# delldu/VSTNet

Hardware: AMD Instinct MI355X
Metric: stylized frames/sec at 1024x1024 (1/2/4/8 GPU) + % HBM roofline (higher is better)
Workload: dtype bf16x3

## Files before the change

include/vstnet.h:

```cpp
#ifndef VSTNET_H
#define VSTNET_H

#include <stddef.h>
#include <stdint.h>

#ifdef __cplusplus
extern "C" {
#endif
#pragma GCC visibility push(default)

#define VST_OK 0
#define VST_E_ARG (-1)
#define VST_E_SHAPE (-2)
#define VST_E_MODE (-3)
#define VST_E_WORKSPACE (-4)

#define VST_PREC_BF16X3 0
#define VST_PREC_FP32 1
#define VST_PREC_F16X2 2

#define VST_PREC_F16X2H 3

#define VST_NUM_BLOCKS 32

// ... 100 lines not shown
                     int Cin, int Cout, int H, int W, int K, int stride, void* stream);
int vst_generic_squeeze(const float* x, float* y, int B, int D, int H, int W, void* stream);
int vst_generic_unsqueeze(const float* y, float* x, int B, int D, int H, int W, void* stream);
int vst_generic_copy_channels(const float* src, float* dst, int B, int C_src, int c0, int n, long HW, int C_dst, int d0,
                              void* stream);
int vst_generic_zero(float* dst, size_t n_floats, void* stream);

size_t vst_cwct_stats_f64_workspace_bytes(int N, long L);
int vst_cwct_stats_f64(const float* x, int N, long L, const uint8_t* mask, int label, double* stats, void* workspace,
                       void* stream);
size_t vst_cwct_factor_f64_workspace_bytes(int N);
int vst_cwct_factor_f64(const double* content_stats, const double* const* style_stats_host_array, const float* alphas_host,
                        int n_styles, float alpha_c, float eps, int N, double* affine, int* info, void* workspace,
                        void* stream);
int vst_cwct_apply_f64(const float* x, float* y, int N, long L, const double* affine, const uint8_t* mask, int label,
                       void* stream);

size_t vst_cwct_stats_n_workspace_bytes(int N, long L);
int vst_cwct_stats_n(const float* x, int N, long L, const uint8_t* mask, int label, double* stats, void* workspace,
                     size_t workspace_bytes, void* stream);
size_t vst_cwct_factor_n_workspace_bytes(int N);
int vst_cwct_factor_n(const double* content_stats, const double* const* style_stats_host_array, const float* alphas_host,
                      int n_styles, float alpha_c, float eps, int N, float* affine, int* info, void* workspace,
                      size_t workspace_bytes, void* stream);
int vst_cwct_prefactor_n(const double* stats, int N, float eps, double* out, int* info, void* workspace, size_t workspace_bytes,
                         void* stream);
int vst_cwct_apply_n(const float* x, float* y, int N, long L, const float* affine, const uint8_t* mask, int label, void* stream);
size_t vst_cwct_stats_n_f64_workspace_bytes(int N, long L);
int vst_cwct_stats_n_f64(const float* x, int N, long L, const uint8_t* mask, int label, double* stats, void* workspace,
                         size_t workspace_bytes, void* stream);
size_t vst_cwct_factor_n_f64_workspace_bytes(int N);
int vst_cwct_factor_n_f64(const double* content_stats, const double* const* style_stats_host_array, const float* alphas_host,
                          int n_styles, float alpha_c, float eps, int N, double* affine, int* info, void* workspace,
                          size_t workspace_bytes, void* stream);
int vst_cwct_apply_n_f64(const float* x, float* y, int N, long L, const double* affine, const uint8_t* mask, int label,
                         void* stream);

#define VST_KERNEL_ID(cin, cout, stride) (((cin) << 16) | ((cout) << 4) | (stride))
#define VST_KERNEL_ALL (-1)
#define VST_KERNEL_PACK 1
#define VST_KERNEL_UNPACK 2
#define VST_KERNEL_SPREAD 3
#define VST_KERNEL_GATHER 4
#define VST_KERNEL_CWCT_STATS 5
#define VST_KERNEL_CWCT_FACTOR 6
#define VST_KERNEL_CWCT_APPLY 7
#define VST_KERNEL_PRESPLIT 8
int vst_profile_begin(int kernel_id, int max_records);
int vst_profile_end(double* total_ms, int* launches);
int vst_profile_end_table(int* ids, double* ms, int* launches, int cap, int* n_ids);

#define VST_OPT_STAGE3_LEAN 1
#define VST_OPT_STAGE3_PINGPONG 2
int vst_set_option(int option, int value);
int vst_get_option(int option);

#pragma GCC visibility pop
#ifdef __cplusplus
}
#endif
#endif
```

vstnet_amd/_lib.py:

```python
from __future__ import annotations

import ctypes as C
import glob
import os
import subprocess

PKG_DIR = os.path.dirname(os.path.abspath(__file__))
REPO_DIR = os.path.dirname(PKG_DIR)
LIB_PATH = os.environ.get("VSTNET_HIP_LIB") or os.path.join(PKG_DIR, "libvstnet_hip.so")
RESOURCES_PATH = os.path.join(PKG_DIR, "libvstnet_hip.resources.txt")
SOURCES = sorted(glob.glob(os.path.join(PKG_DIR, "csrc", "*.hip")))
HEADERS = sorted(glob.glob(os.path.join(PKG_DIR, "csrc", "*.h"))) + [os.path.join(REPO_DIR, "include", "vstnet.h")]

NUM_BLOCKS = 32
PREC_BF16X3 = 0
PREC_FP32 = 1
PREC_F16X2 = 2
PREC_F16X2H = 3

EXPORTS = [
    "vst_version", "vst_error_string", "vst_conv_packed_bytes", "vst_pack_conv", "vst_pack_input",
    "vst_unpack_output", "vst_pack_input_u8", "vst_unpack_output_u8", "vst_revnet_forward_u8", "vst_revnet_inverse_u8",
    "vst_spread", "vst_gather", "vst_block_tmp_bytes", "vst_block_apply",
    "vst_pass_workspace_bytes", "vst_revnet_forward", "vst_revnet_inverse",
    "vst_cwct_stats_workspace_bytes", "vst_cwct_stats", "vst_cwct_factor", "vst_cwct_apply", "vst_cwct_apply_prec",
    "vst_cwct_prefactor", "vst_label_plan", "vst_cwct_labels_workspace_bytes", "vst_cwct_stats_labels",
    "vst_cwct_factor_labels", "vst_cwct_apply_labels", "vst_profile_begin", "vst_profile_end", "vst_profile_end_table", "vst_lab_luminance",
    "vst_revnet_encode", "vst_revnet_encode_u8", "vst_revnet_decode", "vst_revnet_decode_u8", "vst_code_to_z", "vst_z_to_code",
    "vst_cwct_stats_code_workspace_bytes", "vst_cwct_stats_code", "vst_cwct_apply_code",
    "vst_mask_to_code", "vst_cwct_stats_labels_code_workspace_bytes", "vst_cwct_stats_labels_code", "vst_cwct_apply_labels_code",
    "vst_revnet_decode_labels", "vst_revnet_decode_labels_u8", "vst_pass_sub_batch",
    "vst_normalize_block", "vst_range_flags", "vst_range_flags_async",
    "vst_cwct_stats_f64_workspace_bytes", "vst_cwct_stats_f64", "vst_cwct_factor_f64_workspace_bytes", "vst_cwct_factor_f64",
    "vst_cwct_apply_f64",
    "vst_generic_conv", "vst_generic_squeeze", "vst_generic_unsqueeze", "vst_generic_copy_channels", "vst_generic_zero",
    "vst_set_option", "vst_get_option",
    "vst_cwct_stats_n_workspace_bytes", "vst_cwct_stats_n", "vst_cwct_factor_n_workspace_bytes", "vst_cwct_factor_n",
    "vst_cwct_prefactor_n", "vst_cwct_apply_n", "vst_cwct_stats_n_f64_workspace_bytes", "vst_cwct_stats_n_f64",
    "vst_cwct_factor_n_f64_workspace_bytes", "vst_cwct_factor_n_f64", "vst_cwct_apply_n_f64",
]
OPT_STAGE3_LEAN = 1
OPT_STAGE3_PINGPONG = 2
RANGE_SATURATED = 1
RANGE_WEIGHT = 2


PRECISIONS = {"bf16x3": PREC_BF16X3, "fp32": PREC_FP32, "f16x2": PREC_F16X2, "f16x2h": PREC_F16X2H}


def default_precision() -> str:
    p = os.environ.get("VST_PRECISION", "bf16x3")
    if p not in PRECISIONS:
        raise ValueError(f"VST_PRECISION must be one of {sorted(PRECISIONS)}")
    return p


class VstError(RuntimeError):
    pass


class ConvWeights(C.Structure):
    _fields_ = [("packed", C.c_void_p), ("bias", C.c_void_p)]


class BlockWeights(C.Structure):
    _fields_ = [("conv", ConvWeights * 3)]


class NetWeights(C.Structure):
    _fields_ = [("blocks", BlockWeights * NUM_BLOCKS)]


def build(force: bool = False, verbose: bool = False) -> str:
    newest_src = max(os.path.getmtime(p) for p in SOURCES + HEADERS)
    if not force and os.path.exists(LIB_PATH) and os.path.getmtime(LIB_PATH) >= newest_src:
        return LIB_PATH
    hipcc = os.environ.get("HIPCC", "/opt/rocm/bin/hipcc")
    cmd = [hipcc, "-O3", "--offload-arch=gfx950", "-fPIC", "-shared", "-std=c++17", "-Xarch_host", "-fvisibility=hidden",
           "-I", os.path.join(REPO_DIR, "include"), "-o", LIB_PATH] + SOURCES
    cmd[1:1] = ["-Rpass-analysis=kernel-resource-usage", "-fno-caret-diagnostics"]
    if verbose:
        print(" ".join(cmd))
    p = subprocess.run(cmd, stderr=subprocess.PIPE, text=True)
    remarks = [ln.split("remark:", 1)[1].split("[-Rpass")[0].strip() for ln in p.stderr.splitlines() if "remark:" in ln]
    other = "\n".join(ln for ln in p.stderr.splitlines() if "remark:" not in ln and "kernel-resource-usage" not in ln)
    if p.returncode != 0:
        raise subprocess.CalledProcessError(p.returncode, cmd, stderr=other)
    if other.strip():
        print(other)
    table, name = [], None
    for r in remarks:
        if r.startswith("Function Name:"):
            name = r.split(":", 1)[1].strip()
        elif name and (r.startswith("VGPRs:") or r.startswith("ScratchSize") or r.startswith("LDS Size") or r.startswith("Occupancy")):
            table.append(f"{name}\t{r}")
# ... 162 lines not shown
```

vstnet_amd/csrc/conv.hip:

```cpp
#include <mutex>
#include <stdlib.h>
#include "common.h"

#ifndef VST_ABLATE
#define VST_ABLATE 0
#endif

struct ConvArgs {
    const float* in;
    float* out;
    const unsigned char* packed;
    const float* bias;
    int Hin, Win, Hout, Wout;
    int Wq;
    size_t in_img_stride;
    size_t out_img_stride;
    float sign;
    int tiles_x, tiles_y, tiles_total;
    const unsigned char* packed1;
    const float* bias1;
    unsigned char* out_sp;
    size_t out_sp_img_bytes;
    unsigned trace_base;
};
// ... 675 lines not shown
    for (int m = 0; m < C::MR; ++m)
#pragma unroll
        for (int n = 0; n < C::NB; ++n) acc[m][n] = f32x4{0.f, 0.f, 0.f, 0.f};
    const int slot_base = (wave * C::MR) * C::IW + lrow;
#pragma unroll
    for (int ks = 0; ks < C::KS; ++ks) {
        bf16x8 wh[C::NB], wl[C::NB];
#pragma unroll
        for (int n = 0; n < C::NB; ++n) {
            const int boff = ((ks * 4 + kg) * C::NT + n * 16 + lrow) * 16;
            wh[n] = __builtin_bit_cast(bf16x8, *(const uint4*)(b_hi + boff));
            wl[n] = __builtin_bit_cast(bf16x8, *(const uint4*)(b_lo + boff));
        }
#pragma unroll
        for (int m = 0; m < C::MR; ++m) {
            bf16x8 xh, xl;
            read_x_small<MID>(a_hi, a_lo, C::NSLOT, slot_base + m * C::IW, C::IW, ks, kg, xh, xl);
#pragma unroll
            for (int n = 0; n < C::NB; ++n) { MFMA_T(acc[m][n], wh[n], wl[n], xh, xl); }
        }
    }
    load_bias<CH, C::NB>(a, 4 * kg, bias);
    if constexpr (TERMS == 2) vst_note_range(range_amax);
    if (!EARLY_OLD) { PAIR_FETCH_OLD(); }
#undef PAIR_FETCH_OLD
    if (interior) store_tile<CH, true, C::MR, C::NB, true>(a, out_img, ty0 + wave * C::MR, tx0 + lrow, 4 * kg, acc, bias, old);
    else store_tile<CH, true, C::MR, C::NB>(a, out_img, ty0 + wave * C::MR, tx0 + lrow, 4 * kg, acc, bias, old);
    VST_TRACE_END_(1, MID, CH)
}

#ifdef VST_PP_STAMP
__device__ unsigned long long vst_pp_stamps[2 * 32 * 8];
extern "C" __attribute__((visibility("default"))) int vst_pp_stamps_dump(unsigned long long* host) {
    return (int)hipMemcpyFromSymbol(host, HIP_SYMBOL(vst_pp_stamps), sizeof(vst_pp_stamps));
}
#define PP_STAMP(grp_, st_, k_)                                                                                  \
    if (blockIdx.x == 128 && lane == 0 && (wave & 3) == 0 && (st_) < 32) {                                       \
        asm volatile("s_waitcnt lgkmcnt(0)" ::: "memory");                                                      \
        vst_pp_stamps[((grp_) * 32 + (st_)) * 8 + (k_)] = __builtin_amdgcn_s_memtime();                          \
    }
__device__ unsigned long long vst_pp_clk[4];
extern "C" __attribute__((visibility("default"))) int vst_pp_clk_dump(unsigned long long* host) {
    return (int)hipMemcpyFromSymbol(host, HIP_SYMBOL(vst_pp_clk), sizeof(vst_pp_clk));
}
#define PP_CLK(i_)                                                                                               \
    if (blockIdx.x == 128 && threadIdx.x == 0) {                                                                 \
        vst_pp_clk[2 * (i_)] = __builtin_amdgcn_s_memtime();                                                     \
        vst_pp_clk[2 * (i_) + 1] = __builtin_amdgcn_s_memrealtime();                                             \
    }
#else
#define PP_STAMP(grp_, st_, k_)
#define PP_CLK(i_)
#endif
template <int CIN, int COUT, int NW_ = 8>
struct PipeCfg {
    static constexpr int NW = NW_, NTHR = 64 * NW;
    static constexpr int NT = 64, NB = 4, MR = 2, TH = MR * NW, IW = 18, NPIX = (TH + 2) * IW, NSLOT = (NPIX + 15) / 16 * 16;
    static constexpr int NCHUNK = CIN / 32, NCOT = COUT / 64;
    static constexpr int A_PLANE = 4 * NSLOT * 16, A_BUF = 2 * A_PLANE;
    static constexpr int B_PLANE = 3 * 4 * 64 * 16, B_BUF = 2 * B_PLANE;
    static constexpr int LDS_BYTES = 2 * A_BUF + 2 * B_BUF;
    static constexpr int A_PART = NPIX * 4 / 3;
    static constexpr int A_ITEMS = ((A_PART / 4 + 15) / 16 * 64 + NTHR - 1) / NTHR;
    static constexpr int B_ITEMS = 2 * 768 / NTHR;
    static_assert(NPIX % 3 == 0, "three equal parts");
};

template <int CIN, int COUT, bool IN_STATE, bool OUT_STATE, int NW = 8>
__global__ __launch_bounds__(64 * NW, NW == 4 ? 2 : 1) void conv_pipe_kernel(const ConvArgs a) {
    using C = PipeCfg<CIN, COUT, NW>;
    extern __shared__ __attribute__((aligned(16))) unsigned char smem[];
    unsigned char* const Abuf = smem;
    unsigned char* const Bbuf = smem + 2 * C::A_BUF;

    const int tid = threadIdx.x, lane = tid & 63, wave = tid >> 6;
    const int lrow = lane & 15, kg = lane >> 4;
    int bx, by, b;
    if (!xcd_tile(a, bx, by, b)) return;
    VST_TRACE_BEGIN(4)
    PP_CLK(0)
    const int tx0 = bx * 16, ty0 = by * C::TH;
    const float* const in_img = a.in + (size_t)b * a.in_img_stride;
    float* const out_img = a.out + (size_t)b * a.out_img_stride;
    const PackedConvLayout PL = packed_conv_layout(COUT, CIN);
    const unsigned char* const w_plane0 = a.packed + PL.f32_bytes;

    unsigned a_src[3][C::A_ITEMS], a_dst[3][C::A_ITEMS];
#pragma unroll
    for (int part = 0; part < 3; ++part)
#pragma unroll
        for (int it = 0; it < C::A_ITEMS; ++it) {
            const int j = it * C::NTHR + tid;
            int sl = (j >> 6) * 16 + (j & 15);
            sl = sl < C::A_PART / 4 ? sl : C::A_PART / 4 - 1;
            const int cig = (j >> 4) & 3, slot = part * (C::A_PART / 4) + sl;
            const int iy = slot / C::IW, ix = slot - iy * C::IW;
            const int gy = reflect_clamp(ty0 - 1 + iy, a.Hin), gx = reflect_clamp(tx0 - 1 + ix, a.Win);
            const size_t off = IN_STATE ? zc_offset(vst_level_of_channels(CIN), gy, gx, a.Wq)
                                        : ((size_t)gy * a.Win + gx) * CIN;
            a_src[part][it] = (unsigned)(off + cig * 8);
            a_dst[part][it] = (cig * C::NSLOT + slot) * 16;
        }
    typedef f32x4 APart[C::A_ITEMS][2];
    typedef u32x4 BStage[C::B_ITEMS];
#define LOAD_A(r, chunk, part)                                                          \
    _Pragma("unroll") for (int it_ = 0; it_ < C::A_ITEMS; ++it_) {                      \
        const float* p_ = in_img + a_src[part][it_] + (chunk) * 32;                     \
        r[it_][0] = *(const f32x4*)p_; r[it_][1] = *(const f32x4*)(p_ + 4);             \
    }
#define F4_(v_) make_float4((v_)[0], (v_)[1], (v_)[2], (v_)[3])
#define STORE_A(buf, part, r)                                                           \
    _Pragma("unroll") for (int it_ = 0; it_ < C::A_ITEMS; ++it_) {                      \
        unsigned char* base_ = Abuf + (buf) * C::A_BUF;                                 \
        uint4 h_, l_;                                                                   \
        split8(F4_(r[it_][0]), F4_(r[it_][1]), h_, l_);                                 \
        *(uint4*)(base_ + a_dst[part][it_]) = h_;                                       \
        *(uint4*)(base_ + C::A_PLANE + a_dst[part][it_]) = l_;                          \
    }
    int b_off[C::B_ITEMS], b_dst[C::B_ITEMS];
#pragma unroll
    for (int it = 0; it < C::B_ITEMS; ++it) {
        if constexpr (NW == 4) {
            const int plane = it / 3, k3 = it % 3, kgi = tid >> 6, co = tid & 63;
            b_off[it] = ((kgi * COUT + co) * 16) + (int)(plane * PL.frag_bytes) + k3 * 4 * COUT * 16;
            b_dst[it] = tid * 16 + plane * C::B_PLANE + k3 * 256 * 16;
        } else {
            const int idx = it * C::NTHR + tid;
            const int plane = idx >= 768, r = idx - plane * 768;
            const int k3 = r >> 8, kgi = (r >> 6) & 3, co = r & 63;
            b_off[it] = (int)(plane * PL.frag_bytes) + ((k3 * 4 + kgi) * COUT + co) * 16;
            b_dst[it] = plane * C::B_PLANE + r * 16;
        }
    }
#define LOAD_B(r, q_, dy_)                                                              \
    {                                                                                   \
        const int cot_ = (q_) / C::NCHUNK, chunk_ = (q_) - cot_ * C::NCHUNK;            \
        const unsigned char* src_ = w_plane0 + ((size_t)(chunk_ * 9 + (dy_) * 3) * 4 * COUT + cot_ * 64) * 16;   \
        _Pragma("unroll") for (int it_ = 0; it_ < C::B_ITEMS; ++it_) r[it_] = *(const u32x4*)(src_ + b_off[it_]); \
    }
#define STORE_B(buf, r)                                                                 \
    { _Pragma("unroll") for (int it_ = 0; it_ < C::B_ITEMS; ++it_) *(u32x4*)(Bbuf + (buf) * C::B_BUF + b_dst[it_]) = r[it_]; }
    struct Frags { bf16x8 wh[4], wl[4], xh[C::MR], xl[C::MR]; };
    auto read_frags = [&](Frags& f, const unsigned char* Ab, const unsigned char* Bb, int k3) {
#pragma unroll
        for (int n = 0; n < 4; ++n) {
            f.wh[n] = __builtin_bit_cast(bf16x8, *(const uint4*)(Bb + (k3 * 256 + n * 16) * 16));
            f.wl[n] = __builtin_bit_cast(bf16x8, *(const uint4*)(Bb + C::B_PLANE + (k3 * 256 + n * 16) * 16));
        }
#pragma unroll
        for (int m = 0; m < C::MR; ++m) {
            f.xh[m] = __builtin_bit_cast(bf16x8, *(const uint4*)(Ab + (m * C::IW + k3) * 16));
            f.xl[m] = __builtin_bit_cast(bf16x8, *(const uint4*)(Ab + C::A_PLANE + (m * C::IW + k3) * 16));
        }
    };

    constexpr int Q = C::NCOT * C::NCHUNK;
    static_assert(Q % 2 == 0, "stage parity is static only for an even number of (slice, chunk) pairs");
    constexpr bool ONE_SET = NW == 4;
#define RS(i_) (ONE_SET ? 0 : (i_))
    BStage rb[ONE_SET ? 1 : 2];
    APart ra[ONE_SET ? 1 : 2];
    {
        BStage rb0;
        LOAD_B(rb0, 0, 0);
        APart r0, r1, r2;
        LOAD_A(r0, 0, 0); LOAD_A(r1, 0, 1); LOAD_A(r2, 0, 2);
        LOAD_B(rb[RS(1)], 0, 1);
        if (C::NCHUNK > 1) LOAD_A(ra[RS(1)], 1, 0);
        STORE_A(0, 0, r0); STORE_A(0, 1, r1); STORE_A(0, 2, r2);
        STORE_B(0, rb0);
    }
    __syncthreads();

    f32x4 acc[C::MR][4];
#pragma unroll
    for (int m = 0; m < C::MR; ++m)
#pragma unroll
        for (int n = 0; n < 4; ++n) acc[m][n] = f32x4{0.f, 0.f, 0.f, 0.f};
    const int slot_base = (wave * C::MR) * C::IW + lrow;
    const int oy0 = ty0 + wave * C::MR;
    float4 bias[4], old[C::MR][4];
#if VST_ABLATE & 8
    f32x16 abl_big[2];
#pragma unroll
    for (int i = 0; i < 16; ++i) { abl_big[0][i] = 0.f; abl_big[1][i] = 0.f; }
#endif
    const bool full_tile = ty0 + C::TH <= a.Hout && tx0 + 16 <= a.Wout;
    constexpr bool DEFER = OUT_STATE && C::NCOT > 1 && C::NCHUNK == 2 && !VST_PIPE_NO_DEFER;
    bool pending = false;
    int pend_cot = 0;

#pragma unroll 1
    for (int q0 = 0; q0 < Q; q0 += 2) {
#pragma unroll
      for (int qq = 0; qq < 2; ++qq) {
        const int q = q0 + qq;
        const int cot = q / C::NCHUNK, chunk = q - cot * C::NCHUNK;
        const bool last_chunk = chunk == C::NCHUNK - 1;
#pragma unroll
        for (int dy = 0; dy < 3; ++dy) {
            const int s = q * 3 + dy;
            const int cur = (qq * 3 + dy) & 1;
#define PIPE_LAND()                                                                                 \
            if (!(VST_ABLATE & 2)) {                                                                \
                if (s + 1 < 3 * Q) STORE_B((s + 1) & 1, rb[RS(cur ^ 1)]);                            \
                if (q < C::NCHUNK - 1) STORE_A((chunk + 1) & 1, dy, ra[RS(cur ^ 1)]);                \
            }
            if constexpr (ONE_SET) { PIPE_LAND(); }
            if (!(VST_ABLATE & 2)) {
                const int q2 = dy == 0 ? q : q + 1, dy2 = (dy + 2) % 3;
                if (q2 < Q) LOAD_B(rb[RS(cur)], q2, dy2);
                const int qn = dy == 2 ? q + 1 : q, dyn = (dy + 1) % 3;
                if (qn < C::NCHUNK - 1) LOAD_A(ra[RS(cur)], qn + 1, dyn);
            }
            if (DEFER ? (dy == 2 && last_chunk) : (dy == 0 && chunk == 0)) load_bias<COUT, 4>(a, cot * 64 + 4 * kg, bias);
            if (OUT_STATE && !(DEFER && VST_PIPE_OLD_SPREAD) && dy == 2 && last_chunk && (!(VST_ABLATE & 4) || cot == C::NCOT - 1)) {
                if (full_tile) load_old<COUT, C::MR, 4, true>(a, out_img, oy0, tx0 + lrow, cot * 64 + 4 * kg, old);
                else load_old<COUT, C::MR, 4, false>(a, out_img, oy0, tx0 + lrow, cot * 64 + 4 * kg, old);
            }

            if constexpr (!ONE_SET) { PIPE_LAND(); }
#undef PIPE_LAND

            const unsigned char* Ab = Abuf + (chunk & 1) * C::A_BUF + (kg * C::NSLOT + slot_base + dy * C::IW) * 16;
            const unsigned char* Bb = Bbuf + (s & 1) * C::B_BUF + (kg * 64 + lrow) * 16;
            Frags fr[2];
            read_frags(fr[0], Ab, Bb, 0);
#pragma unroll
            for (int k3 = 0; k3 < 3; ++k3) {
                __builtin_amdgcn_sched_barrier(0);
                if (k3 < 2 && !(VST_ABLATE & 1)) read_frags(fr[(k3 + 1) & 1], Ab, Bb, k3 + 1);
                if constexpr (DEFER) {
                    if (qq == 0 && dy * 3 + k3 < C::MR * 4) {
                        const int unit = dy * 3 + k3, m_ = unit >> 2, n_ = unit & 3;
                        if (pending) {
                            float4* p_ = full_tile ? out_ptr<COUT, OUT_STATE, true>(a, out_img, oy0 + m_, tx0 + lrow, pend_cot * 64 + 4 * kg + n_ * 16)
                                                   : out_ptr<COUT, OUT_STATE, false>(a, out_img, oy0 + m_, tx0 + lrow, pend_cot * 64 + 4 * kg + n_ * 16);
                            if (full_tile || p_) *p_ = old[m_][n_];
                        }
                        if (VST_PIPE_OLD_SPREAD) {
                            const float4* q_ = full_tile ? out_ptr<COUT, OUT_STATE, true>(a, out_img, oy0 + m_, tx0 + lrow, cot * 64 + 4 * kg + n_ * 16)
                                                         : out_ptr<COUT, OUT_STATE, false>(a, out_img, oy0 + m_, tx0 + lrow, cot * 64 + 4 * kg + n_ * 16);
                            old[m_][n_] = (full_tile || q_) ? *q_ : make_float4(0.f, 0.f, 0.f, 0.f);
                        }
                    }
                }
                __builtin_amdgcn_sched_barrier(0);
                const Frags& f = fr[(VST_ABLATE & 1) ? 0 : (k3 & 1)];
#if VST_ABLATE & 8
#pragma unroll
                for (int jb = 0; jb < 2; ++jb) {
                    abl_big[jb] = __builtin_amdgcn_mfma_f32_32x32x16_bf16(f.wh[2 * jb], f.xl[0], abl_big[jb], 0, 0, 0);
                    abl_big[jb] = __builtin_amdgcn_mfma_f32_32x32x16_bf16(f.wl[2 * jb], f.xh[0], abl_big[jb], 0, 0, 0);
                    abl_big[jb] = __builtin_amdgcn_mfma_f32_32x32x16_bf16(f.wh[2 * jb], f.xh[0], abl_big[jb], 0, 0, 0);
                    abl_big[jb] = __builtin_amdgcn_mfma_f32_32x32x16_bf16(f.wh[2 * jb + 1], f.xl[1], abl_big[jb], 0, 0, 0);
                    abl_big[jb] = __builtin_amdgcn_mfma_f32_32x32x16_bf16(f.wl[2 * jb + 1], f.xh[1], abl_big[jb], 0, 0, 0);
                    abl_big[jb] = __builtin_amdgcn_mfma_f32_32x32x16_bf16(f.wh[2 * jb + 1], f.xh[1], abl_big[jb], 0, 0, 0);
                }
#else
#pragma unroll
                for (int m = 0; m < C::MR; ++m)
#pragma unroll
                    for (int n = 0; n < 4; ++n) { MFMA3(acc[m][n], f.wh[n], f.wl[n], f.xh[m], f.xl[m]); }
#endif
            }

            if (DEFER && dy == 2 && last_chunk && cot != C::NCOT - 1 && !(VST_ABLATE & 4)) {
#pragma unroll
                for (int m = 0; m < C::MR; ++m)
#pragma unroll
                    for (int n = 0; n < 4; ++n) {
                        const float4 o = old[m][n];
                        old[m][n] = make_float4(o.x + a.sign * (acc[m][n][0] + bias[n].x), o.y + a.sign * (acc[m][n][1] + bias[n].y),
                                                o.z + a.sign * (acc[m][n][2] + bias[n].z), o.w + a.sign * (acc[m][n][3] + bias[n].w));
                        acc[m][n] = f32x4{0.f, 0.f, 0.f, 0.f};
                    }
                pending = true;
                pend_cot = cot;
            } else
            if (dy == 2 && last_chunk && (!(VST_ABLATE & 4) || cot == C::NCOT - 1)) {
                if (full_tile) store_tile<COUT, OUT_STATE, C::MR, 4, true>(a, out_img, oy0, tx0 + lrow, cot * 64 + 4 * kg, acc, bias, old);
                else store_tile<COUT, OUT_STATE, C::MR, 4, false>(a, out_img, oy0, tx0 + lrow, cot * 64 + 4 * kg, acc, bias, old);
#pragma unroll
                for (int m = 0; m < C::MR; ++m)
#pragma unroll
                    for (int n = 0; n < 4; ++n) acc[m][n] = f32x4{0.f, 0.f, 0.f, 0.f};
            }
            if (DEFER && qq == 0 && dy == 2) pending = false;
            if ((VST_ABLATE & 4) && dy == 2 && last_chunk && cot != C::NCOT - 1) {
#pragma unroll
                for (int m = 0; m < C::MR; ++m)
#pragma unroll
                    for (int n = 0; n < 4; ++n) asm volatile("" : "+v"(acc[m][n]));
            }
            if (!(VST_ABLATE & 16)) __syncthreads();
        }
      }
    }
#undef LOAD_A
#undef STORE_A
#undef LOAD_B
#undef STORE_B
#undef F4_
#undef RS
#if VST_ABLATE & 8
    asm volatile("" :: "v"(abl_big[0]), "v"(abl_big[1]));
#endif
    PP_CLK(1)
    VST_TRACE_END_(4, CIN, COUT)
}

#ifndef VST_WITH_PINGPONG
#define VST_WITH_PINGPONG 0
#endif
#if VST_WITH_PINGPONG
template <int CIN, int COUT, bool IN_STATE, bool OUT_STATE>
__global__ __launch_bounds__(512) void conv_pp_kernel(const ConvArgs a) {
    using C = PipeCfg<CIN, COUT, 8>;
    constexpr int SY = 256;
    constexpr int A_ITEMS_Y = ((C::A_PART / 4 + 15) / 16 * 64 + SY - 1) / SY;
    constexpr int B_ITEMS_Y = 2 * 768 / SY;
    extern __shared__ __attribute__((aligned(16))) unsigned char smem[];
    unsigned char* const Abuf = smem;
    unsigned char* const Bbuf = smem + 2 * C::A_BUF;
    float* const bias_lds = (float*)(smem + C::LDS_BYTES);

    const int tid = threadIdx.x, lane = tid & 63, wave = __builtin_amdgcn_readfirstlane(tid >> 6);
    const int lrow = lane & 15, kg = lane >> 4;
    const bool grpY = wave >= 4;
    int bx, by, b;
    if (!xcd_tile(a, bx, by, b)) return;
    VST_TRACE_BEGIN(4)
    PP_CLK(0)
    const int tx0 = bx * 16, ty0 = by * C::TH;
    const float* const in_img = a.in + (size_t)b * a.in_img_stride;
    float* const out_img = a.out + (size_t)b * a.out_img_stride;
    const PackedConvLayout PL = packed_conv_layout(COUT, CIN);
    const unsigned char* const w_plane0 = a.packed + PL.f32_bytes;
    constexpr int Q = C::NCOT * C::NCHUNK, S = 3 * Q;
    constexpr bool A_IN_LOOP = C::NCHUNK > 2;

#define PP_A_ADDR(j_, part_, src_, dst_)                                                                         \
    {                                                                                                            \
        int sl_ = ((j_) >> 6) * 16 + ((j_) & 15);                                                                \
        sl_ = sl_ < C::A_PART / 4 ? sl_ : C::A_PART / 4 - 1;                                                     \
        const int cig_ = ((j_) >> 4) & 3, slot_ = (part_) * (C::A_PART / 4) + sl_;                               \
        const int iy_ = slot_ / C::IW, ix_ = slot_ - iy_ * C::IW;                                                \
        const int gy_ = reflect_clamp(ty0 - 1 + iy_, a.Hin), gx_ = reflect_clamp(tx0 - 1 + ix_, a.Win);          \
        const size_t off_ = IN_STATE ? zc_offset(vst_level_of_channels(CIN), gy_, gx_, a.Wq)                     \
                                     : ((size_t)gy_ * a.Win + gx_) * CIN;                                        \
        src_ = (unsigned)(off_ + cig_ * 8);                                                                      \
        dst_ = (cig_ * C::NSLOT + slot_) * 16;                                                                   \
    }
#define PP_F4(v_) make_float4((v_)[0], (v_)[1], (v_)[2], (v_)[3])
#define PP_LAND_A(base_, r0_, r1_, dst_)                                                                         \
    {                                                                                                            \
        uint4 h_, l_;                                                                                            \
// ... 256 lines not shown
        size_t rest = idx / COUT;
        const int ox = rest % a.Wout; rest /= a.Wout;
        const int oy = rest % a.Hout;
        const int b = rest / a.Hout;
        const float* in_img = a.in + (size_t)b * a.in_img_stride;
        float acc = a.bias[co];
        for (int tap = 0; tap < 9; ++tap) {
            const int gy = reflect_clamp(oy * STRIDE - 1 + tap / 3, a.Hin);
            const int gx = reflect_clamp(ox * STRIDE - 1 + tap % 3, a.Win);
            const float* p = in_img + (IN_STATE ? zc_offset(vst_level_of_channels(CIN), gy, gx, a.Wq)
                                                : ((size_t)gy * a.Win + gx) * CIN);
            const float* w = wf + (size_t)tap * CIN * COUT + co;
            for (int ci = 0; ci < CIN; ++ci) acc = fmaf(p[ci], w[(size_t)ci * COUT], acc);
        }
        float* out_img = a.out + (size_t)b * a.out_img_stride;
        if (OUT_STATE) {
            float* p = out_img + zc_offset(vst_level_of_channels(COUT), oy, ox, a.Wq) + co;
            *p = *p + a.sign * acc;
        } else {
            out_img[((size_t)oy * a.Wout + ox) * COUT + co] = acc > 0.f ? acc : 0.f;
        }
    }
}

#define VST_PROFILE_MAX_RECORDS 4096
static std::mutex g_prof_mu;
static std::atomic<int> g_prof_kernel{0};
static int g_prof_count = 0, g_prof_cap = 0;
static int g_prof_id[VST_PROFILE_MAX_RECORDS];
static hipEvent_t g_prof_ev[2 * VST_PROFILE_MAX_RECORDS];
static bool g_prof_ev_created = false;

int vst_prof_open(int kernel_id, hipStream_t st) {
    const int sel = g_prof_kernel.load(std::memory_order_relaxed);
    if (sel != kernel_id && sel != VST_KERNEL_ALL) return -1;
    std::lock_guard<std::mutex> lk(g_prof_mu);
    if ((g_prof_kernel.load() != kernel_id && g_prof_kernel.load() != VST_KERNEL_ALL) || g_prof_count >= g_prof_cap) return -1;
    const int rec = g_prof_count++;
    g_prof_id[rec] = kernel_id;
    (void)hipEventRecord(g_prof_ev[2 * rec], st);
    return rec;
}

void vst_prof_close(int rec, hipStream_t st) {
    std::lock_guard<std::mutex> lk(g_prof_mu);
    if (rec < g_prof_count) (void)hipEventRecord(g_prof_ev[2 * rec + 1], st);
}

#ifndef VST_LEAN_DEFAULT
#define VST_LEAN_DEFAULT 0
#endif
static std::atomic<int> g_opt_lean{[] { const char* e = getenv("VST_LEAN"); return e && (e[0] == '0' || e[0] == '1') ? e[0] - '0' : VST_LEAN_DEFAULT; }()};
static bool vst_lean_stage3() { return g_opt_lean.load(std::memory_order_relaxed) != 0; }
#ifndef VST_PINGPONG_DEFAULT
#define VST_PINGPONG_DEFAULT 0
#endif
static std::atomic<int> g_opt_pp{[] { const char* e = getenv("VST_PINGPONG"); return e && (e[0] == '0' || e[0] == '1') ? e[0] - '0' : VST_PINGPONG_DEFAULT; }()};

template <int CIN, int COUT, int STRIDE, bool IN_STATE, bool OUT_STATE>
static int launch_conv(const ConvArgs& a, int B, int precision, hipStream_t st, bool out_h16 = false) {
    if (precision == VST_PREC_FP32) {
        const size_t total = (size_t)B * a.Hout * a.Wout * COUT;
        size_t blocks = (total + 255) / 256;
        if (blocks > 65536) blocks = 65536;
        conv_fp32_kernel<IN_STATE, OUT_STATE><<<dim3((unsigned)blocks), 256, 0, st>>>(a, CIN, COUT, STRIDE, B);
        VST_RETURN_IF_LAUNCH_FAILED();
        return VST_OK;
    }
    if (precision != VST_PREC_BF16X3 && !vst_is_f16(precision)) return VST_E_MODE;
    vst_prof_scope prof(VST_KERNEL_ID(CIN, COUT, STRIDE), st);
    if constexpr (CIN >= 64 && COUT >= 64 && STRIDE == 1) {
        ConvArgs t = a;
        t.tiles_x = (a.Wout + 15) / 16;
        if (vst_lean_stage3()) {
            using C = PipeCfg<CIN, COUT, 4>;
            auto kern = conv_pipe_kernel<CIN, COUT, IN_STATE, OUT_STATE, 4>;
            static std::atomic<unsigned> attr_done{0};
            if (int rc_ = vst_ensure_dynamic_lds((const void*)kern, (int)(C::LDS_BYTES), &attr_done)) return rc_;
            t.tiles_y = (a.Hout + C::TH - 1) / C::TH; t.tiles_total = t.tiles_x * t.tiles_y * B;
            VST_TRACE_RESERVE(t, (t.tiles_total + 7) / 8 * 8)
            kern<<<dim3((t.tiles_total + 7) / 8 * 8), C::NTHR, C::LDS_BYTES, st>>>(t);
#if VST_WITH_PINGPONG
        } else if (g_opt_pp.load(std::memory_order_relaxed)) {
            using C = PipeCfg<CIN, COUT>;
            auto kern = conv_pp_kernel<CIN, COUT, IN_STATE, OUT_STATE>;
            constexpr int lds = C::LDS_BYTES + (OUT_STATE ? COUT * 4 : 0);
            static std::atomic<unsigned> attr_done{0};
            if (int rc_ = vst_ensure_dynamic_lds((const void*)kern, lds, &attr_done)) return rc_;
            t.tiles_y = (a.Hout + C::TH - 1) / C::TH; t.tiles_total = t.tiles_x * t.tiles_y * B;
            VST_TRACE_RESERVE(t, (t.tiles_total + 7) / 8 * 8)
            kern<<<dim3((t.tiles_total + 7) / 8 * 8), C::NTHR, lds, st>>>(t);
#endif
        } else {
            using C = PipeCfg<CIN, COUT>;
            auto kern = conv_pipe_kernel<CIN, COUT, IN_STATE, OUT_STATE>;
            static std::atomic<unsigned> attr_done{0};
            if (int rc_ = vst_ensure_dynamic_lds((const void*)kern, (int)(C::LDS_BYTES), &attr_done)) return rc_;
            t.tiles_y = (a.Hout + C::TH - 1) / C::TH; t.tiles_total = t.tiles_x * t.tiles_y * B;
            VST_TRACE_RESERVE(t, (t.tiles_total + 7) / 8 * 8)
            kern<<<dim3((t.tiles_total + 7) / 8 * 8), C::NTHR, C::LDS_BYTES, st>>>(t);
        }
    } else {
        using C = ConvCfg<CIN, COUT, STRIDE>;
        constexpr bool T2_SHAPE = (CIN == 64 && COUT == 16) || (CIN == 16 && COUT == 16 && STRIDE == 2) || (CIN == 16 && COUT == 4);
        const bool t2 = T2_SHAPE && vst_is_f16(precision);
        constexpr bool H16_SHAPE = T2_SHAPE && !OUT_STATE;
        const bool h16 = t2 && out_h16 && H16_SHAPE;
        auto kern = h16 ? conv_mfma_kernel<CIN, COUT, STRIDE, IN_STATE, OUT_STATE, false, T2_SHAPE ? 2 : 3, H16_SHAPE>
                  : t2 ? conv_mfma_kernel<CIN, COUT, STRIDE, IN_STATE, OUT_STATE, false, T2_SHAPE ? 2 : 3>
                       : conv_mfma_kernel<CIN, COUT, STRIDE, IN_STATE, OUT_STATE, false, 3>;
        const int lds = t2 ? C::LDS_BYTES_T2 : C::LDS_BYTES;
        static std::atomic<unsigned> attr_done[3];
        if (int rc_ = vst_ensure_dynamic_lds((const void*)kern, lds, &attr_done[h16 ? 2 : (t2 ? 1 : 0)])) return rc_;
        ConvArgs t = a;
        t.tiles_x = (a.Wout + C::TW - 1) / C::TW; t.tiles_y = (a.Hout + C::TH - 1) / C::TH;
        t.tiles_total = t.tiles_x * t.tiles_y * B * C::NCOT;
        VST_TRACE_RESERVE(t, (t.tiles_total + 7) / 8 * 8)
        kern<<<dim3((t.tiles_total + 7) / 8 * 8), 256, lds, st>>>(t);
    }
    VST_RETURN_IF_LAUNCH_FAILED();
    return VST_OK;
}

static int launch_conv_s2_planes(const ConvArgs& a, int B, hipStream_t st) {
    using C = ConvCfg<64, 64, 2>;
    vst_prof_scope prof(VST_KERNEL_ID(64, 64, 2), st);
    auto kern = conv_mfma_kernel<64, 64, 2, true, false, true, 2>;
    static std::atomic<unsigned> attr_done{0};
    if (int rc_ = vst_ensure_dynamic_lds((const void*)kern, (int)(C::LDS_BYTES_T2), &attr_done)) return rc_;
// ... 64 lines not shown
    a.in = src; a.out = h1; a.packed = (const unsigned char*)w->conv[0].packed; a.bias = w->conv[0].bias;
    a.Hin = Ho * STRIDE; a.Win = Wo * STRIDE; a.Hout = Ho; a.Wout = Wo;
    a.in_img_stride = state_img; a.out_img_stride = mid_img; a.sign = 0.f;
    if constexpr (CH == 256 && STRIDE == 2) {
        if (vst_is_f16(precision)) {
            const size_t mid_bytes = (size_t)Ho * Wo * 64 * 4, state_bytes = (size_t)Ho * Wo * 256 * 4;
            unsigned char* const h1p = (unsigned char*)tmp;
            unsigned char* const h2p = h1p + (size_t)B * mid_bytes;
            unsigned char* const planes_a = h2p + (size_t)B * mid_bytes;
            (void)state_bytes;
            a.out_sp = h1p; a.out_sp_img_bytes = mid_bytes;
            int rc2 = launch_conv_s2_planes(a, B, st);
            if (rc2) return rc2;
            const int h2_single = precision == VST_PREC_F16X2H;
            rc2 = vst3_conv_mid(&w->conv[1], h1p, h2p, h2_single, B, H, W, st);
            if (rc2) return rc2;
            return vst3_conv_out(&w->conv[2], h2p, h2_single, dst, direction > 0 ? planes_a : nullptr, direction > 0 ? 1.f : -1.f,
                                 B, H, W, st);
        }
    }
    const bool h16 = CH <= 64 && VST_PAIR && precision == VST_PREC_F16X2H;
    int rc = launch_conv<IN_CH, MID, STRIDE, true, false>(a, B, precision, st, h16);
    if (rc) return rc;
    if constexpr (CH <= 64 && VST_PAIR) {
        if (precision != VST_PREC_FP32) {
            a.in = h1; a.out = dst; a.Hin = Ho; a.Win = Wo; a.in_img_stride = mid_img; a.out_img_stride = state_img;
            a.packed = (const unsigned char*)w->conv[2].packed; a.bias = w->conv[2].bias;
            a.packed1 = (const unsigned char*)w->conv[1].packed; a.bias1 = w->conv[1].bias;
            a.sign = direction > 0 ? 1.f : -1.f;
            return launch_pair<MID, CH>(a, B, precision, st);
        }
    }
    a.in = h1; a.out = h2; a.packed = (const unsigned char*)w->conv[1].packed; a.bias = w->conv[1].bias;
    a.Hin = Ho; a.Win = Wo; a.in_img_stride = mid_img;
    rc = launch_conv<MID, MID, 1, false, false>(a, B, precision, st);
    if (rc) return rc;
    a.in = h2; a.out = dst; a.packed = (const unsigned char*)w->conv[2].packed; a.bias = w->conv[2].bias;
    a.out_img_stride = state_img; a.sign = direction > 0 ? 1.f : -1.f;
    return launch_conv<MID, CH, 1, false, true>(a, B, precision, st);
}

static const int kBlockChannel[VST_NUM_BLOCKS] = {16, 16, 16, 16, 16, 16, 16, 16, 16, 16, 64, 64, 64, 64, 64, 64,
                                                  64, 64, 64, 64, 256, 256, 256, 256, 256, 256, 256, 256, 256, 256,
                                                  256, 256};
static const int kBlockStride[VST_NUM_BLOCKS] = {1, 1, 1, 1, 1, 1, 1, 1, 1, 1, 2, 1, 1, 1, 1, 1,
                                                 1, 1, 1, 1, 2, 1, 1, 1, 1, 1, 1, 1, 1, 1, 1, 1};

VST_DEFINE_TU_RANGE(vst_range_tu_conv)

extern "C" {

int vst_set_option(int option, int value) {
    if (option == VST_OPT_STAGE3_LEAN) g_opt_lean.store(value != 0, std::memory_order_relaxed);
    else if (option == VST_OPT_STAGE3_PINGPONG && VST_WITH_PINGPONG) g_opt_pp.store(value != 0, std::memory_order_relaxed);
    else return VST_E_ARG;
    return VST_OK;
}

int vst_get_option(int option) {
    if (option == VST_OPT_STAGE3_LEAN) return g_opt_lean.load(std::memory_order_relaxed);
    if (option == VST_OPT_STAGE3_PINGPONG && VST_WITH_PINGPONG) return g_opt_pp.load(std::memory_order_relaxed);
    return VST_E_ARG;
}

int vst_range_flags(unsigned* flags_host, int reset) {
    if (!flags_host) return VST_E_ARG;
    hipError_t e = hipDeviceSynchronize();
    if (e != hipSuccess) return (int)e;
    unsigned v = 0;
    if (int rc = vst_range_tu_conv(&v, reset)) return rc;
    if (int rc = vst_range_tu_conv3(&v, reset)) return rc;
    if (int rc = vst_range_tu_layout(&v, reset)) return rc;
    if (int rc = vst_range_tu_cwct(&v, reset)) return rc;
    *flags_host = v;
    return VST_OK;
}

int vst_range_flags_async(unsigned* flags4_dev, void* stream) {
    if (!flags4_dev) return VST_E_ARG;
    hipStream_t st = (hipStream_t)stream;
    if (int rc = vst_range_tu_conv_async(flags4_dev + 0, st)) return rc;
    if (int rc = vst_range_tu_conv3_async(flags4_dev + 1, st)) return rc;
    if (int rc = vst_range_tu_layout_async(flags4_dev + 2, st)) return rc;
    return vst_range_tu_cwct_async(flags4_dev + 3, st);
}

int vst_profile_begin(int kernel_id, int max_records) {
    if ((kernel_id <= 0 && kernel_id != VST_KERNEL_ALL) || max_records <= 0) return VST_E_ARG;
    if (max_records > VST_PROFILE_MAX_RECORDS) max_records = VST_PROFILE_MAX_RECORDS;
    std::lock_guard<std::mutex> lk(g_prof_mu);
    if (!g_prof_ev_created) {
        for (int i = 0; i < 2 * VST_PROFILE_MAX_RECORDS; ++i) {
            hipError_t e = hipEventCreate(&g_prof_ev[i]);
            if (e != hipSuccess) return (int)e;
        }
        g_prof_ev_created = true;
    }
    g_prof_count = 0; g_prof_cap = max_records;
    g_prof_kernel.store(kernel_id);
    return VST_OK;
}

int vst_profile_end(double* total_ms, int* launches) {
    if (!total_ms || !launches) return VST_E_ARG;
    std::lock_guard<std::mutex> lk(g_prof_mu);
    g_prof_kernel.store(0);
    double tot = 0.0;
    for (int i = 0; i < g_prof_count; ++i) {
        hipError_t e = hipEventSynchronize(g_prof_ev[2 * i + 1]);
        if (e != hipSuccess) return (int)e;
        float ms = 0.f;
        e = hipEventElapsedTime(&ms, g_prof_ev[2 * i], g_prof_ev[2 * i + 1]);
        if (e != hipSuccess) return (int)e;
// ... 316 lines not shown
```

Before: 207.8.

## Add wide 4-wave stage-3 conv variant with four rows per wave

Adds a WIDE configuration of the pipelined conv kernel (4 waves, MR=4 rows each) that keeps the tile height of the 8-wave kernel while halving the wave count, so each wave reuses its weight fragments across more output rows. The LDS and global staging loads are interleaved explicitly with the MFMAs through sched_group_barrier patterns, and deferred output writes are split into paired units. This path is on by default when lean mode is off. It trades occupancy and register pressure (larger accumulator arrays, one block per CU) for less per-wave B-fragment traffic.

```diff
diff --git a/include/vstnet.h b/include/vstnet.h
--- a/include/vstnet.h
+++ b/include/vstnet.h
@@ -176,6 +176,7 @@
 
 #define VST_OPT_STAGE3_LEAN 1
 #define VST_OPT_STAGE3_PINGPONG 2
+#define VST_OPT_STAGE3_WIDE 3
 int vst_set_option(int option, int value);
 int vst_get_option(int option);
 
diff --git a/vstnet_amd/_lib.py b/vstnet_amd/_lib.py
--- a/vstnet_amd/_lib.py
+++ b/vstnet_amd/_lib.py
@@ -41,6 +41,7 @@
 ]
 OPT_STAGE3_LEAN = 1
 OPT_STAGE3_PINGPONG = 2
+OPT_STAGE3_WIDE = 3
 RANGE_SATURATED = 1
 RANGE_WEIGHT = 2
 
diff --git a/vstnet_amd/csrc/conv.hip b/vstnet_amd/csrc/conv.hip
--- a/vstnet_amd/csrc/conv.hip
+++ b/vstnet_amd/csrc/conv.hip
@@ -751,10 +751,10 @@
 #define PP_STAMP(grp_, st_, k_)
 #define PP_CLK(i_)
 #endif
-template <int CIN, int COUT, int NW_ = 8>
+template <int CIN, int COUT, int NW_ = 8, int MR_ = 2>
 struct PipeCfg {
-    static constexpr int NW = NW_, NTHR = 64 * NW;
-    static constexpr int NT = 64, NB = 4, MR = 2, TH = MR * NW, IW = 18, NPIX = (TH + 2) * IW, NSLOT = (NPIX + 15) / 16 * 16;
+    static constexpr int NW = NW_, NTHR = 64 * NW, MR = MR_;
+    static constexpr int NT = 64, NB = 4, TH = MR * NW, IW = 18, NPIX = (TH + 2) * IW, NSLOT = (NPIX + 15) / 16 * 16;
     static constexpr int NCHUNK = CIN / 32, NCOT = COUT / 64;
     static constexpr int A_PLANE = 4 * NSLOT * 16, A_BUF = 2 * A_PLANE;
     static constexpr int B_PLANE = 3 * 4 * 64 * 16, B_BUF = 2 * B_PLANE;
@@ -763,11 +763,24 @@
     static constexpr int A_ITEMS = ((A_PART / 4 + 15) / 16 * 64 + NTHR - 1) / NTHR;
     static constexpr int B_ITEMS = 2 * 768 / NTHR;
     static_assert(NPIX % 3 == 0, "three equal parts");
+    static_assert(LDS_BYTES <= 160 * 1024, "LDS budget");
 };
 
-template <int CIN, int COUT, bool IN_STATE, bool OUT_STATE, int NW = 8>
-__global__ __launch_bounds__(64 * NW, NW == 4 ? 2 : 1) void conv_pipe_kernel(const ConvArgs a) {
-    using C = PipeCfg<CIN, COUT, NW>;
+template <int NDSR, int NVM, int NDW>
+__device__ __forceinline__ void wide_interleave() {
+#pragma unroll
+    for (int i = 0; i < 48; ++i) {
+        __builtin_amdgcn_sched_group_barrier(0x008, 1, 0);
+        if (i % 2 == 0 && i / 2 < NDSR) __builtin_amdgcn_sched_group_barrier(0x100, 1, 0);
+        if (i % 2 == 1 && i / 2 < NVM) __builtin_amdgcn_sched_group_barrier(0x020, 1, 0);
+        if (i % 2 == 1 && i / 2 < NDW) __builtin_amdgcn_sched_group_barrier(0x200, 1, 0);
+    }
+}
+
+template <int CIN, int COUT, bool IN_STATE, bool OUT_STATE, int NW = 8, int MR = 2>
+__global__ __launch_bounds__(64 * NW, (NW == 4 && MR == 2) ? 2 : 1) void conv_pipe_kernel(const ConvArgs a) {
+    using C = PipeCfg<CIN, COUT, NW, MR>;
+    constexpr bool WIDE = NW == 4 && MR == 4;
     extern __shared__ __attribute__((aligned(16))) unsigned char smem[];
     unsigned char* const Abuf = smem;
     unsigned char* const Bbuf = smem + 2 * C::A_BUF;
@@ -855,7 +868,7 @@
 
     constexpr int Q = C::NCOT * C::NCHUNK;
     static_assert(Q % 2 == 0, "stage parity is static only for an even number of (slice, chunk) pairs");
-    constexpr bool ONE_SET = NW == 4;
+    constexpr bool ONE_SET = NW == 4 && !WIDE;
 #define RS(i_) (ONE_SET ? 0 : (i_))
     BStage rb[ONE_SET ? 1 : 2];
     APart ra[ONE_SET ? 1 : 2];
@@ -888,6 +901,20 @@
     constexpr bool DEFER = OUT_STATE && C::NCOT > 1 && C::NCHUNK == 2 && !VST_PIPE_NO_DEFER;
     bool pending = false;
     int pend_cot = 0;
+#define DEFER_UNIT(unit_)                                                                                                             \
+    {                                                                                                                                 \
+        const int m_ = (unit_) >> 2, n_ = (unit_) & 3;                                                                                \
+        if (pending) {                                                             \
+            float4* p_ = full_tile ? out_ptr<COUT, OUT_STATE, true>(a, out_img, oy0 + m_, tx0 + lrow, pend_cot * 64 + 4 * kg + n_ * 16) \
+                                   : out_ptr<COUT, OUT_STATE, false>(a, out_img, oy0 + m_, tx0 + lrow, pend_cot * 64 + 4 * kg + n_ * 16); \
+            if (full_tile || p_) *p_ = old[m_][n_];                                                                                   \
+        }                                                                                                                             \
+        if (VST_PIPE_OLD_SPREAD) {                                             \
+            const float4* q_ = full_tile ? out_ptr<COUT, OUT_STATE, true>(a, out_img, oy0 + m_, tx0 + lrow, cot * 64 + 4 * kg + n_ * 16) \
+                                         : out_ptr<COUT, OUT_STATE, false>(a, out_img, oy0 + m_, tx0 + lrow, cot * 64 + 4 * kg + n_ * 16); \
+            old[m_][n_] = (full_tile || q_) ? *q_ : make_float4(0.f, 0.f, 0.f, 0.f);                                                  \
+        }                                                                                                                             \
+    }
 
 #pragma unroll 1
     for (int q0 = 0; q0 < Q; q0 += 2) {
@@ -900,6 +927,48 @@
         for (int dy = 0; dy < 3; ++dy) {
             const int s = q * 3 + dy;
             const int cur = (qq * 3 + dy) & 1;
+            if constexpr (WIDE) {
+                constexpr bool A_ALWAYS = C::NCOT == 1;
+                const int q2 = dy == 0 ? q : q + 1, dy2 = (dy + 2) % 3;
+                const int qn = dy == 2 ? q + 1 : q, dyn = (dy + 1) % 3;
+                if (DEFER ? (dy == 2 && last_chunk) : (dy == 0 && chunk == 0)) load_bias<COUT, 4>(a, cot * 64 + 4 * kg, bias);
+                if (!A_ALWAYS && q < C::NCHUNK - 1) STORE_A((chunk + 1) & 1, dy, ra[cur ^ 1]);
+                if (!A_ALWAYS && qn < C::NCHUNK - 1) LOAD_A(ra[cur], qn + 1, dyn);
+                if (OUT_STATE && !(DEFER && VST_PIPE_OLD_SPREAD) && dy == 2 && last_chunk) {
+                    if (full_tile) load_old<COUT, C::MR, 4, true>(a, out_img, oy0, tx0 + lrow, cot * 64 + 4 * kg, old);
+                    else load_old<COUT, C::MR, 4, false>(a, out_img, oy0, tx0 + lrow, cot * 64 + 4 * kg, old);
+                }
+                const unsigned char* Ab = Abuf + (chunk & 1) * C::A_BUF + (kg * C::NSLOT + slot_base + dy * C::IW) * 16;
+                const unsigned char* Bb = Bbuf + (s & 1) * C::B_BUF + (kg * 64 + lrow) * 16;
+                Frags fr[2];
+#pragma unroll
+                for (int k3 = 0; k3 < 3; ++k3) {
+                    if constexpr (DEFER) {
+                        if (qq == 0 && dy * 3 + k3 < C::MR * 2) { DEFER_UNIT(2 * (dy * 3 + k3)); DEFER_UNIT(2 * (dy * 3 + k3) + 1); }
+                    }
+                    if (k3 == 0) read_frags(fr[0], Ab, Bb, 0);
+                    __builtin_amdgcn_sched_barrier(0);
+                    if (k3 == 0) {
+                        LOAD_B(rb[cur], q2 < Q ? q2 : Q - 1, dy2);
+                        if (A_ALWAYS) LOAD_A(ra[cur], qn + 1 < C::NCHUNK ? qn + 1 : C::NCHUNK - 1, dyn);
+                    }
+                    if (k3 < 2) read_frags(fr[(k3 + 1) & 1], Ab, Bb, k3 + 1);
+                    if (k3 == 2) {
+                        STORE_B((s + 1) & 1, rb[cur ^ 1]);
+                        if (A_ALWAYS) STORE_A((chunk + 1) & 1, dy, ra[cur ^ 1]);
+                    }
+                    const Frags& f = fr[k3 & 1];
+#pragma unroll
+                    for (int m = 0; m < C::MR; ++m)
+#pragma unroll
+                        for (int n = 0; n < 4; ++n) { MFMA3(acc[m][n], f.wh[n], f.wl[n], f.xh[m], f.xl[m]); }
+                    constexpr int NSTG = A_ALWAYS ? C::B_ITEMS + 2 * C::A_ITEMS : C::B_ITEMS;
+                    if (k3 == 0) wide_interleave<16, NSTG, 0>();
+                    else if (k3 == 1) wide_interleave<16, 0, 0>();
+                    else wide_interleave<0, 0, NSTG>();
+                    __builtin_amdgcn_sched_barrier(0);
+                }
+            } else {
 #define PIPE_LAND()                                                                                 \
             if (!(VST_ABLATE & 2)) {                                                                \
                 if (s + 1 < 3 * Q) STORE_B((s + 1) & 1, rb[RS(cur ^ 1)]);                            \
@@ -930,19 +999,7 @@
                 __builtin_amdgcn_sched_barrier(0);
                 if (k3 < 2 && !(VST_ABLATE & 1)) read_frags(fr[(k3 + 1) & 1], Ab, Bb, k3 + 1);
                 if constexpr (DEFER) {
-                    if (qq == 0 && dy * 3 + k3 < C::MR * 4) {
-                        const int unit = dy * 3 + k3, m_ = unit >> 2, n_ = unit & 3;
-                        if (pending) {
-                            float4* p_ = full_tile ? out_ptr<COUT, OUT_STATE, true>(a, out_img, oy0 + m_, tx0 + lrow, pend_cot * 64 + 4 * kg + n_ * 16)
-                                                   : out_ptr<COUT, OUT_STATE, false>(a, out_img, oy0 + m_, tx0 + lrow, pend_cot * 64 + 4 * kg + n_ * 16);
-                            if (full_tile || p_) *p_ = old[m_][n_];
-                        }
-                        if (VST_PIPE_OLD_SPREAD) {
-                            const float4* q_ = full_tile ? out_ptr<COUT, OUT_STATE, true>(a, out_img, oy0 + m_, tx0 + lrow, cot * 64 + 4 * kg + n_ * 16)
-                                                         : out_ptr<COUT, OUT_STATE, false>(a, out_img, oy0 + m_, tx0 + lrow, cot * 64 + 4 * kg + n_ * 16);
-                            old[m_][n_] = (full_tile || q_) ? *q_ : make_float4(0.f, 0.f, 0.f, 0.f);
-                        }
-                    }
+                    if (qq == 0 && dy * 3 + k3 < C::MR * 4) DEFER_UNIT(dy * 3 + k3);
                 }
                 __builtin_amdgcn_sched_barrier(0);
                 const Frags& f = fr[(VST_ABLATE & 1) ? 0 : (k3 & 1)];
@@ -962,6 +1019,7 @@
 #pragma unroll
                     for (int n = 0; n < 4; ++n) { MFMA3(acc[m][n], f.wh[n], f.wl[n], f.xh[m], f.xl[m]); }
 #endif
+            }
             }
 
             if (DEFER && dy == 2 && last_chunk && cot != C::NCOT - 1 && !(VST_ABLATE & 4)) {
@@ -1002,6 +1060,7 @@
 #undef STORE_B
 #undef F4_
 #undef RS
+#undef DEFER_UNIT
 #if VST_ABLATE & 8
     asm volatile("" :: "v"(abl_big[0]), "v"(abl_big[1]));
 #endif
@@ -1364,6 +1423,10 @@
 #endif
 static std::atomic<int> g_opt_lean{[] { const char* e = getenv("VST_LEAN"); return e && (e[0] == '0' || e[0] == '1') ? e[0] - '0' : VST_LEAN_DEFAULT; }()};
 static bool vst_lean_stage3() { return g_opt_lean.load(std::memory_order_relaxed) != 0; }
+#ifndef VST_WIDE_DEFAULT
+#define VST_WIDE_DEFAULT 1
+#endif
+static std::atomic<int> g_opt_wide{[] { const char* e = getenv("VST_WIDE"); return e && (e[0] == '0' || e[0] == '1') ? e[0] - '0' : VST_WIDE_DEFAULT; }()};
 #ifndef VST_PINGPONG_DEFAULT
 #define VST_PINGPONG_DEFAULT 0
 #endif
@@ -1387,6 +1450,14 @@
         if (vst_lean_stage3()) {
             using C = PipeCfg<CIN, COUT, 4>;
             auto kern = conv_pipe_kernel<CIN, COUT, IN_STATE, OUT_STATE, 4>;
+            static std::atomic<unsigned> attr_done{0};
+            if (int rc_ = vst_ensure_dynamic_lds((const void*)kern, (int)(C::LDS_BYTES), &attr_done)) return rc_;
+            t.tiles_y = (a.Hout + C::TH - 1) / C::TH; t.tiles_total = t.tiles_x * t.tiles_y * B;
+            VST_TRACE_RESERVE(t, (t.tiles_total + 7) / 8 * 8)
+            kern<<<dim3((t.tiles_total + 7) / 8 * 8), C::NTHR, C::LDS_BYTES, st>>>(t);
+        } else if (g_opt_wide.load(std::memory_order_relaxed)) {
+            using C = PipeCfg<CIN, COUT, 4, 4>;
+            auto kern = conv_pipe_kernel<CIN, COUT, IN_STATE, OUT_STATE, 4, 4>;
             static std::atomic<unsigned> attr_done{0};
             if (int rc_ = vst_ensure_dynamic_lds((const void*)kern, (int)(C::LDS_BYTES), &attr_done)) return rc_;
             t.tiles_y = (a.Hout + C::TH - 1) / C::TH; t.tiles_total = t.tiles_x * t.tiles_y * B;
@@ -1557,6 +1628,7 @@
 
 int vst_set_option(int option, int value) {
     if (option == VST_OPT_STAGE3_LEAN) g_opt_lean.store(value != 0, std::memory_order_relaxed);
+    else if (option == VST_OPT_STAGE3_WIDE) g_opt_wide.store(value != 0, std::memory_order_relaxed);
     else if (option == VST_OPT_STAGE3_PINGPONG && VST_WITH_PINGPONG) g_opt_pp.store(value != 0, std::memory_order_relaxed);
     else return VST_E_ARG;
     return VST_OK;
@@ -1564,6 +1636,7 @@
 
 int vst_get_option(int option) {
     if (option == VST_OPT_STAGE3_LEAN) return g_opt_lean.load(std::memory_order_relaxed);
+    if (option == VST_OPT_STAGE3_WIDE) return g_opt_wide.load(std::memory_order_relaxed);
     if (option == VST_OPT_STAGE3_PINGPONG && VST_WITH_PINGPONG) return g_opt_pp.load(std::memory_order_relaxed);
     return VST_E_ARG;
 }
```

Result: faster. 214.2 (median of 6 runs) (+3.1%).
